# diegoferigo/gym-ignition

Hardware: AMD Instinct MI355X
Metric: env·steps/sec (whole node) at N parallel worlds; obs max-abs-err vs DART (higher is better)
Workload: dtype f32

## Files before the change

### gym-ignition_amd/csrc/group_kernel.hip

```cpp
#include "group_tree.hpp"
#include "kernels.hpp"
#include "rng.hpp"
#include "xcd.hpp"

namespace mw {
namespace dev {

#ifdef MW_GROUP_PROF
__device__ unsigned long long g_group_prof[kGroupProfPhases];
#endif

template <int N, bool DUAL, bool CONS>
__global__ void __launch_bounds__(64) vecenv_pid_group_kernel(const ChainF* __restrict__ P, TaskF T, SimDev S,
                                                              VecDev V, const GLaneTask* __restrict__ lt,
                                                              const float* __restrict__ targets,
                                                              float* __restrict__ obs, float* __restrict__ reward,
                                                              uint8_t* __restrict__ done_out,
                                                              float* __restrict__ term_obs, int W, int n, float dt,
                                                              float inv_dt, int substeps, int pgs_iters) {
    unsigned long long prof[kGroupProfPhases] = {};
    MW_GPROF_T(k0);
    const int li = static_cast<int>(threadIdx.x) & (kGroupLanes - 1);
    const int wb = xcd_block();
    const int wr = static_cast<int>((wb * blockDim.x + threadIdx.x) / kGroupLanes);
    const bool live = wr < W;
    const int w = live ? wr : W - 1;
    const bool body = li < n;
    const GBody<N> B = load_gbody<N>(P, li, n);
    const GTopo TT = load_gtopo(P);
    PidF g{};
    float home = 0.f;
    if (body) {
        g = lt[li].pid;
        home = lt[li].home;
    }
    const f3 grav = {P->g[0], P->g[1], P->g[2]};
    const int dl = body ? li : 0;
    float q = 0.f, qd = 0.f, qlo = 0.f, tgt = 0.f, pe = 0.f, pi = 0.f, pu = 0.f;
    if (body) {
        q = S.q[dl * W + w];
        qd = S.qd[dl * W + w];
        qlo = S.qlo[dl * W + w];
        tgt = targets[static_cast<size_t>(w) * n + dl];
        pe = S.pid_e[dl * W + w];
        pi = S.pid_i[dl * W + w];
        pu = S.pid_u[dl * W + w];
    }
    const uint32_t episode0 = V.episode[w];
    const uint32_t steps0 = V.steps[w];
    MW_GPROF_T(k1);
    MW_GPROF_ACC(0, k0, k1);
    for (int s = 0; s < substeps; ++s) {
        float tau = 0.f;
        if (body) {
            float u = pu;
            if (!pid_update(g, (q - tgt) + qlo, inv_dt, dt, pe, pi, u)) u = 0.f;
            else pu = u;
            tau = fminf(fmaxf(u, -B.effort), B.effort);
        }
        group_substep<N, DUAL, CONS>(B, li, n, TT, grav, q, qd, qlo, tau, dt, inv_dt, pgs_iters,
                                     prof);
    }
    MW_GPROF_T(k2);
    const float e = body ? (q - tgt) * (q - tgt) : 0.f;
    float r = 0.f;
    sfor<N>([&](auto D) { r -= row_bcast<D>(e); });
    uint32_t steps = steps0 + 1u;
    const bool d_ = (T.max_steps > 0 && steps >= static_cast<uint32_t>(T.max_steps));
    if (live && li == 0) {
        reward[w] = r;
        done_out[w] = d_ ? 1 : 0;
    }
    const size_t ob = static_cast<size_t>(w) * 2 * n;
    if (d_) {
        if (live && body) {
            term_obs[ob + li] = q;
            term_obs[ob + n + li] = qd;
        }
        steps = 0u;
        if (live && li == 0) V.episode[w] = episode0 + 1u;
        uint32_t rr[4];
        philox(T.seed_lo, T.seed_hi, T.world_offset + static_cast<uint32_t>(w), episode0 + 1u, rr,
               static_cast<uint32_t>(li >> 2));
        const int k = li & 3;
        const uint32_t x4 = (k == 0) ? rr[0] : (k == 1) ? rr[1] : (k == 2) ? rr[2] : rr[3];
        const float x = home + unif(x4, -T.home_noise, T.home_noise);
        q = B.limited ? fminf(fmaxf(x, B.lower), B.upper) : x;
        qd = 0.f;
        pe = pi = pu = qlo = 0.f;
    }
    if (live && body) {
        obs[ob + li] = q;
        obs[ob + n + li] = qd;
        S.q[dl * W + w] = q;
        S.qd[dl * W + w] = qd;
        S.qlo[dl * W + w] = qlo;
        S.pid_e[dl * W + w] = pe;
        S.pid_i[dl * W + w] = pi;
        S.pid_u[dl * W + w] = pu;
    }
    if (live && li == 0) V.steps[w] = steps;
#ifdef MW_GROUP_PROF
    MW_GPROF_T(k3);
    MW_GPROF_ACC(7, k2, k3);
    MW_GPROF_ACC(8, k0, k3);
    if (live && li == 0)
        for (int k = 0; k < kGroupProfPhases; ++k) atomicAdd(&g_group_prof[k], prof[k]);
#else
    (void)prof;
#endif
}

}

#ifdef MW_GROUP_PROF
extern "C" int mw_debug_group_prof(unsigned long long* out) {
    if (hipMemcpyFromSymbol(out, HIP_SYMBOL(dev::g_group_prof), sizeof(dev::g_group_prof)) != hipSuccess) return 1;
    const unsigned long long z[dev::kGroupProfPhases] = {};
    return hipMemcpyToSymbol(HIP_SYMBOL(dev::g_group_prof), z, sizeof(z)) == hipSuccess ? 0 : 1;
}
#endif

namespace {
template <int N>
hipError_t group_n(const ChainF* P, int n, bool cons, bool dual, const TaskF& T, const SimDev& S, const VecDev& V,
                   const GLaneTask* pid, const float* targets, float* obs, float* reward, uint8_t* done, float* term_obs,
                   int W, float dt, int substeps, int pgs, hipStream_t st) {
    const dim3 grid(static_cast<unsigned>((W + 3) / 4)), block(64);
    const float inv_dt = 1.f / dt;
    if (!cons)
        hipLaunchKernelGGL((dev::vecenv_pid_group_kernel<N, false, false>), grid, block, 0, st, P, T, S, V, pid,
                           targets, obs, reward, done, term_obs, W, n, dt, inv_dt, substeps, pgs);
    else if (!dual)
        hipLaunchKernelGGL((dev::vecenv_pid_group_kernel<N, false, true>), grid, block, 0, st, P, T, S, V, pid,
                           targets, obs, reward, done, term_obs, W, n, dt, inv_dt, substeps, pgs);
    else
        hipLaunchKernelGGL((dev::vecenv_pid_group_kernel<N, true, true>), grid, block, 0, st, P, T, S, V, pid,
                           targets, obs, reward, done, term_obs, W, n, dt, inv_dt, substeps, pgs);
    return hipGetLastError();
}
}

hipError_t launch_vecenv_pid_group(const ChainF* P, int n, bool cons, bool dual, const TaskF& T, const SimDev& S,
                                   const VecDev& V, const GLaneTask* pid, const float* targets, float* obs,
                                   float* reward, uint8_t* done, float* term_obs, int W, float dt, int substeps,
                                   int pgs_iters, hipStream_t st) {
    if (n < 1 || n > kMaxKernelDofs || W < 1) return hipErrorInvalidValue;
    if (n <= 9)
        return group_n<9>(P, n, cons, dual, T, S, V, pid, targets, obs, reward, done, term_obs, W, dt, substeps,
                          pgs_iters, st);
    return group_n<kMaxKernelDofs>(P, n, cons, dual, T, S, V, pid, targets, obs, reward, done, term_obs, W, dt,
                                   substeps, pgs_iters, st);
}

}
```

### gym-ignition_amd/csrc/xcd.hpp

```cpp
#pragma once

#include <hip/hip_runtime.h>

namespace mw {
namespace dev {

__device__ __forceinline__ int xcd_block() {
    const int nb = static_cast<int>(gridDim.x), bx = static_cast<int>(blockIdx.x);
    const int q = nb >> 3, r = nb & 7, x = bx & 7;
    return x * q + (x < r ? x : r) + (bx >> 3);
}

}
}
```

Baseline: 1.957 billion.

## Pack group kernel arguments into flat kernarg lines and defer tail-argument loads

New measurement: 1.957 billion. Within noise of the previous version (-0.0%).

```diff
diff --git a/gym-ignition_amd/csrc/group_kernel.hip b/gym-ignition_amd/csrc/group_kernel.hip
--- a/gym-ignition_amd/csrc/group_kernel.hip
+++ b/gym-ignition_amd/csrc/group_kernel.hip
@@ -10,47 +10,104 @@
 __device__ unsigned long long g_group_prof[kGroupProfPhases];
 #endif
 
+struct GroupArgs {
+    int32_t substeps, pgs_iters;
+    float* obs;
+    float* reward;
+    uint8_t* done;
+    float* term_obs;
+    int32_t max_steps;
+    uint32_t seed_lo, seed_hi;
+    uint32_t world_offset;
+    float home_noise;
+    int32_t pad_;
+};
+struct GroupFlat {
+    const ChainF* P;
+    const GLaneTask* lt;
+    float* sq;
+    float* spid;
+    const float* targets;
+    uint32_t* cnt;
+    int32_t W, n;
+    float dt, inv_dt;
+};
+struct GroupKernargs {
+    GroupFlat F;
+    GroupArgs A;
+};
+static_assert(sizeof(GroupFlat) == 64, "the flat arguments are one kernarg line (14 of its dwords are preloaded)");
+static_assert(sizeof(GroupArgs) == 64 && alignof(GroupArgs) == 8, "one kernarg line, directly behind the flat arguments");
+static_assert(sizeof(GroupKernargs) <= 192, "the group kernel's kernargs stay within 192 bytes");
+
+template <class E>
+__device__ __forceinline__ auto global_ptr(E* p) {
+    return (__attribute__((address_space(1))) E*)p;
+}
+
+__device__ __forceinline__ GroupKernargs tail_args(float after) {
+    auto kp = reinterpret_cast<uintptr_t>(__builtin_amdgcn_kernarg_segment_ptr());
+    asm volatile("" : "+s"(kp) : "v"(after));
+    const auto* p = reinterpret_cast<const __attribute__((address_space(4))) uint32_t*>(kp);
+    uint32_t v[sizeof(GroupKernargs) / 4];
+#pragma unroll
+    for (unsigned k = 0; k < sizeof(GroupKernargs) / 4; ++k) v[k] = p[k];
+    GroupKernargs t;
+    __builtin_memcpy(&t, v, sizeof(t));
+    return t;
+}
+
 template <int N, bool DUAL, bool CONS>
-__global__ void __launch_bounds__(64) vecenv_pid_group_kernel(const ChainF* __restrict__ P, TaskF T, SimDev S,
-                                                              VecDev V, const GLaneTask* __restrict__ lt,
+__global__ void __launch_bounds__(64) vecenv_pid_group_kernel(const ChainF* __restrict__ P,
+                                                              const GLaneTask* __restrict__ lt,
+                                                              float* __restrict__ sq, float* __restrict__ spid,
                                                               const float* __restrict__ targets,
-                                                              float* __restrict__ obs, float* __restrict__ reward,
-                                                              uint8_t* __restrict__ done_out,
-                                                              float* __restrict__ term_obs, int W, int n, float dt,
-                                                              float inv_dt, int substeps, int pgs_iters) {
+                                                              uint32_t* __restrict__ cnt, int W, int n, float dt,
+                                                              float inv_dt, GroupArgs A) {
     unsigned long long prof[kGroupProfPhases] = {};
     MW_GPROF_T(k0);
-    const int li = static_cast<int>(threadIdx.x) & (kGroupLanes - 1);
-    const int wb = xcd_block();
-    const int wr = static_cast<int>((wb * blockDim.x + threadIdx.x) / kGroupLanes);
+    const GTopo TT = load_gtopo(P);
+    const f3 grav = {P->g[0], P->g[1], P->g[2]};
+    const int tid = static_cast<int>(threadIdx.x);
+    const int li = tid & (kGroupLanes - 1);
+    const int wb = xcd_block((W + 3) >> 2);
+    const int wr = wb * (64 / kGroupLanes) + (tid >> 4);
+    static_assert(kGroupLanes == 16);
     const bool live = wr < W;
     const int w = live ? wr : W - 1;
     const bool body = li < n;
+    const size_t nw = static_cast<size_t>(n) * static_cast<size_t>(W);
+    float* __restrict__ sqd = sq + nw;
+    float* __restrict__ spid_i = spid + nw;
+    float* __restrict__ spid_u = spid + 2 * nw;
+    float* __restrict__ sqlo = spid + 3 * nw;
+    uint32_t* __restrict__ ssteps = cnt + W;
+    const int dl = body ? li : 0;
+    const int si = dl * W + w;
+    const float q_ = sq[si], qd_ = sqd[si], qlo_ = sqlo[si];
+    const float tgt_ = targets[static_cast<size_t>(w) * n + dl];
+    const float pe_ = spid[si], pi_ = spid_i[si], pu_ = spid_u[si];
+    const uint32_t episode0 = cnt[w];
+    const uint32_t steps0 = ssteps[w];
+    const GLaneTask lane = lt[dl];
+    uint32_t model[sizeof(BodyF) / 4];
+    {
+        const uint32_t* __restrict__ mb = reinterpret_cast<const uint32_t*>(&P->b[dl]);
+#pragma unroll
+        for (unsigned k = 0; k < sizeof(BodyF) / 4; ++k) model[k] = mb[k];
+    }
     const GBody<N> B = load_gbody<N>(P, li, n);
-    const GTopo TT = load_gtopo(P);
-    PidF g{};
-    float home = 0.f;
-    if (body) {
-        g = lt[li].pid;
-        home = lt[li].home;
-    }
-    const f3 grav = {P->g[0], P->g[1], P->g[2]};
-    const int dl = body ? li : 0;
-    float q = 0.f, qd = 0.f, qlo = 0.f, tgt = 0.f, pe = 0.f, pi = 0.f, pu = 0.f;
-    if (body) {
-        q = S.q[dl * W + w];
-        qd = S.qd[dl * W + w];
-        qlo = S.qlo[dl * W + w];
-        tgt = targets[static_cast<size_t>(w) * n + dl];
-        pe = S.pid_e[dl * W + w];
-        pi = S.pid_i[dl * W + w];
-        pu = S.pid_u[dl * W + w];
-    }
-    const uint32_t episode0 = V.episode[w];
-    const uint32_t steps0 = V.steps[w];
+#pragma unroll
+    for (unsigned k = 0; k < sizeof(BodyF) / 4; ++k) asm volatile("" ::"v"(model[k]));
+    asm volatile("" ::"s"(A.substeps), "s"(A.pgs_iters));
+    asm volatile("" ::"s"(TT.steps), "s"(TT.levels), "s"(TT.ref), "s"(grav.x), "s"(grav.y), "s"(grav.z));
+    const PidF g = lane.pid;
+    const float home = body ? lane.home : 0.f;
+    float q = body ? q_ : 0.f, qd = body ? qd_ : 0.f, qlo = body ? qlo_ : 0.f, tgt = body ? tgt_ : 0.f;
+    float pe = body ? pe_ : 0.f, pi = body ? pi_ : 0.f, pu = body ? pu_ : 0.f;
     MW_GPROF_T(k1);
     MW_GPROF_ACC(0, k0, k1);
-    for (int s = 0; s < substeps; ++s) {
+    for (int s = 0; s < A.substeps; ++s) {
         float tau = 0.f;
         if (body) {
             float u = pu;
@@ -58,27 +115,39 @@
             else pu = u;
             tau = fminf(fmaxf(u, -B.effort), B.effort);
         }
-        group_substep<N, DUAL, CONS>(B, li, n, TT, grav, q, qd, qlo, tau, dt, inv_dt, pgs_iters,
+        group_substep<N, DUAL, CONS>(B, li, n, TT, grav, q, qd, qlo, tau, dt, inv_dt, A.pgs_iters,
                                      prof);
     }
     MW_GPROF_T(k2);
+    const GroupKernargs K = tail_args(q);
+    const GroupArgs& T = K.A;
     const float e = body ? (q - tgt) * (q - tgt) : 0.f;
     float r = 0.f;
     sfor<N>([&](auto D) { r -= row_bcast<D>(e); });
+    asm volatile("" ::"s"(T.obs), "s"(T.reward), "s"(T.done), "s"(T.term_obs), "s"(T.max_steps), "s"(T.seed_lo),
+                 "s"(T.seed_hi), "s"(T.world_offset), "s"(T.home_noise), "s"(K.F.sq), "s"(K.F.spid), "s"(K.F.cnt),
+                 "s"(K.F.W));
+    int sj = si, wj = w;
+    asm volatile("" : "+v"(sj), "+v"(wj));
+    const size_t nwj = static_cast<size_t>(n) * static_cast<size_t>(K.F.W);
+    const auto tq = global_ptr(K.F.sq), tpid = global_ptr(K.F.spid);
+    const auto tcnt = global_ptr(K.F.cnt);
+    const auto tobs = global_ptr(T.obs), treward = global_ptr(T.reward), tterm = global_ptr(T.term_obs);
+    const auto tdone = global_ptr(T.done);
     uint32_t steps = steps0 + 1u;
     const bool d_ = (T.max_steps > 0 && steps >= static_cast<uint32_t>(T.max_steps));
     if (live && li == 0) {
-        reward[w] = r;
-        done_out[w] = d_ ? 1 : 0;
-    }
-    const size_t ob = static_cast<size_t>(w) * 2 * n;
+        treward[wj] = r;
+        tdone[wj] = d_ ? 1 : 0;
+    }
+    const size_t ob = static_cast<size_t>(wj) * 2 * n;
     if (d_) {
         if (live && body) {
-            term_obs[ob + li] = q;
-            term_obs[ob + n + li] = qd;
+            tterm[ob + li] = q;
+            tterm[ob + n + li] = qd;
         }
         steps = 0u;
-        if (live && li == 0) V.episode[w] = episode0 + 1u;
+        if (live && li == 0) tcnt[wj] = episode0 + 1u;
         uint32_t rr[4];
         philox(T.seed_lo, T.seed_hi, T.world_offset + static_cast<uint32_t>(w), episode0 + 1u, rr,
                static_cast<uint32_t>(li >> 2));
@@ -90,16 +159,16 @@
         pe = pi = pu = qlo = 0.f;
     }
     if (live && body) {
-        obs[ob + li] = q;
-        obs[ob + n + li] = qd;
-        S.q[dl * W + w] = q;
-        S.qd[dl * W + w] = qd;
-        S.qlo[dl * W + w] = qlo;
-        S.pid_e[dl * W + w] = pe;
-        S.pid_i[dl * W + w] = pi;
-        S.pid_u[dl * W + w] = pu;
-    }
-    if (live && li == 0) V.steps[w] = steps;
+        tobs[ob + li] = q;
+        tobs[ob + n + li] = qd;
+        tq[sj] = q;
+        tq[nwj + sj] = qd;
+        tpid[3 * nwj + sj] = qlo;
+        tpid[sj] = pe;
+        tpid[nwj + sj] = pi;
+        tpid[2 * nwj + sj] = pu;
+    }
+    if (live && li == 0) tcnt[K.F.W + wj] = steps;
 #ifdef MW_GROUP_PROF
     MW_GPROF_T(k3);
     MW_GPROF_ACC(7, k2, k3);
@@ -122,21 +191,32 @@
 #endif
 
 namespace {
+struct GroupCall {
+    const ChainF* P;
+    const GLaneTask* lt;
+    float* sq;
+    float* spid;
+    const float* targets;
+    uint32_t* cnt;
+    int W, n;
+    float dt;
+    dev::GroupArgs A;
+    hipStream_t st;
+};
+
 template <int N>
-hipError_t group_n(const ChainF* P, int n, bool cons, bool dual, const TaskF& T, const SimDev& S, const VecDev& V,
-                   const GLaneTask* pid, const float* targets, float* obs, float* reward, uint8_t* done, float* term_obs,
-                   int W, float dt, int substeps, int pgs, hipStream_t st) {
-    const dim3 grid(static_cast<unsigned>((W + 3) / 4)), block(64);
-    const float inv_dt = 1.f / dt;
+hipError_t group_n(bool cons, bool dual, const GroupCall& c) {
+    const dim3 grid(static_cast<unsigned>((c.W + 3) / 4)), block(64);
+    const float inv_dt = 1.f / c.dt;
     if (!cons)
-        hipLaunchKernelGGL((dev::vecenv_pid_group_kernel<N, false, false>), grid, block, 0, st, P, T, S, V, pid,
-                           targets, obs, reward, done, term_obs, W, n, dt, inv_dt, substeps, pgs);
+        hipLaunchKernelGGL((dev::vecenv_pid_group_kernel<N, false, false>), grid, block, 0, c.st, c.P, c.lt, c.sq,
+                           c.spid, c.targets, c.cnt, c.W, c.n, c.dt, inv_dt, c.A);
     else if (!dual)
-        hipLaunchKernelGGL((dev::vecenv_pid_group_kernel<N, false, true>), grid, block, 0, st, P, T, S, V, pid,
-                           targets, obs, reward, done, term_obs, W, n, dt, inv_dt, substeps, pgs);
+        hipLaunchKernelGGL((dev::vecenv_pid_group_kernel<N, false, true>), grid, block, 0, c.st, c.P, c.lt, c.sq,
+                           c.spid, c.targets, c.cnt, c.W, c.n, c.dt, inv_dt, c.A);
     else
-        hipLaunchKernelGGL((dev::vecenv_pid_group_kernel<N, true, true>), grid, block, 0, st, P, T, S, V, pid,
-                           targets, obs, reward, done, term_obs, W, n, dt, inv_dt, substeps, pgs);
+        hipLaunchKernelGGL((dev::vecenv_pid_group_kernel<N, true, true>), grid, block, 0, c.st, c.P, c.lt, c.sq,
+                           c.spid, c.targets, c.cnt, c.W, c.n, c.dt, inv_dt, c.A);
     return hipGetLastError();
 }
 }
@@ -146,11 +226,20 @@
                                    float* reward, uint8_t* done, float* term_obs, int W, float dt, int substeps,
                                    int pgs_iters, hipStream_t st) {
     if (n < 1 || n > kMaxKernelDofs || W < 1) return hipErrorInvalidValue;
-    if (n <= 9)
-        return group_n<9>(P, n, cons, dual, T, S, V, pid, targets, obs, reward, done, term_obs, W, dt, substeps,
-                          pgs_iters, st);
-    return group_n<kMaxKernelDofs>(P, n, cons, dual, T, S, V, pid, targets, obs, reward, done, term_obs, W, dt,
-                                   substeps, pgs_iters, st);
-}
-
-}
+    const size_t nw = static_cast<size_t>(n) * static_cast<size_t>(W);
+    if (S.qd != S.q + nw || S.pid_i != S.pid_e + nw || S.pid_u != S.pid_e + 2 * nw || S.qlo != S.pid_e + 3 * nw ||
+        V.steps != V.episode + W)
+        return hipErrorInvalidValue;
+    dev::GroupArgs A{};
+    A.obs = obs; A.reward = reward; A.done = done; A.term_obs = term_obs;
+    A.substeps = substeps; A.pgs_iters = pgs_iters;
+    A.max_steps = T.max_steps;
+    A.seed_lo = T.seed_lo; A.seed_hi = T.seed_hi;
+    A.world_offset = T.world_offset;
+    A.home_noise = T.home_noise;
+    const GroupCall c{P, pid, S.q, S.pid_e, targets, V.episode, W, n, dt, A, st};
+    if (n <= 9) return group_n<9>(cons, dual, c);
+    return group_n<kMaxKernelDofs>(cons, dual, c);
+}
+
+}
diff --git a/gym-ignition_amd/csrc/xcd.hpp b/gym-ignition_amd/csrc/xcd.hpp
--- a/gym-ignition_amd/csrc/xcd.hpp
+++ b/gym-ignition_amd/csrc/xcd.hpp
@@ -5,11 +5,13 @@
 namespace mw {
 namespace dev {
 
-__device__ __forceinline__ int xcd_block() {
-    const int nb = static_cast<int>(gridDim.x), bx = static_cast<int>(blockIdx.x);
+__device__ __forceinline__ int xcd_block(int nb) {
+    const int bx = static_cast<int>(blockIdx.x);
     const int q = nb >> 3, r = nb & 7, x = bx & 7;
     return x * q + (x < r ? x : r) + (bx >> 3);
 }
 
+__device__ __forceinline__ int xcd_block() { return xcd_block(static_cast<int>(gridDim.x)); }
+
 }
 }
```
